# jgrss/cultionet

Hardware: AMD Instinct MI355X
Metric: train_chips_per_sec (higher is better)
Workload: dtype f32

## Files before the change

### cultionet_amd/csrc/cn_thin.hip

```cpp
#include "cn_common.h"

namespace {

struct Taps {
  int off[9];
  bool ok[9];
};

__device__ __forceinline__ Taps cn_thin_taps(int oy, int ox, int H, int W, int dil, int sgn) {
  Taps tp;
#pragma unroll
  for (int t = 0; t < 9; ++t) {
    const int iy = oy + sgn * (t / 3 - 1) * dil, ix = ox + sgn * (t % 3 - 1) * dil;
    tp.ok[t] = iy >= 0 && iy < H && ix >= 0 && ix < W;
    tp.off[t] = tp.ok[t] ? iy * W + ix : 0;
  }
  return tp;
}

#define CN_THIN_W(g) ((g) == 0 ? w0 : ((g) == 1 ? w1 : w2))
#define CN_THIN_B(g) ((g) == 0 ? b0 : ((g) == 1 ? b1 : b2))
#define CN_THIN_DW(g) ((g) == 0 ? dw0 : ((g) == 1 ? dw1 : dw2))

template <int NG, int CP, bool GROUPED>
// ... 262 lines not shown
#pragma unroll
    for (int u = 0; u < U; ++u) {
      if (c0 + u < Cq) {
        const int cw = wid * Cq + c0 + u;
        const float* wrow = wpk ? wpk + (long)(cw < Cin ? cw : 0) * RS : wl + cw * RS;
        const bool wok = !wpk || cw < Cin;
        const int wa = wok ? __float_as_int(wrow[lane]) : 0;
        const int wb = wok ? __float_as_int(wrow[64 + (lane < RS - 64 ? lane : 0)]) : 0;
#pragma unroll
        for (int o = 0; o < NO; ++o)
#pragma unroll
          for (int t = 0; t < 9; ++t) {
            const int i = o * 9 + t;
            acc[o] = fmaf(xv[u][t], __int_as_float(__builtin_amdgcn_readlane(i < 64 ? wa : wb, i & 63)), acc[o]);
          }
      }
    }
  }
#pragma unroll
  for (int o = 0; o < NO; ++o) red[(wid * NO + o) * 64 + lane] = acc[o];
  __syncthreads();
  for (int idx = threadIdx.x; idx < NO * 64; idx += 256) {
    const int o = idx >> 6, l = idx & 63;
    const int g = o / CP, c = o - g * CP;
    const float* bg = g == 0 ? b0 : (g == 1 ? b1 : b2);
    float v = bg != nullptr ? bg[c] : 0.f;
#pragma unroll
    for (int w = 0; w < 4; ++w) v += red[(w * NO + o) * 64 + l];
    const int p = bx * 64 + l;
    if (p < HW) y[(long)by * ybs + (long)o * HW + p] = v;
  }
}

template <int NG, int CP>
__global__ __launch_bounds__(256) void cn_thin_bwd_data_ks_kernel(const float* __restrict__ dy, long dybs,
                                                                 const float* __restrict__ w0,
                                                                 const float* __restrict__ w1,
                                                                 const float* __restrict__ w2,
                                                                 float* __restrict__ dx, long dxbs, int Cin, int H,
                                                                 int W, int dil, int accumulate, int Cq, int B,
                                                                 const float* __restrict__ wpk) {
  constexpr int NO = NG * CP, RS = (NO * 9 + 3) / 4 * 4;
  extern __shared__ __attribute__((aligned(16))) float sm[];
  float* wl = sm;
  const int lane = threadIdx.x & 63, wid = threadIdx.x >> 6;
  const int HW = H * W;
  int bx, by, bz;
  const int gx = (HW + 63) / 64;
  if (!cn_xcd_block(gx, B, gx * B, bx, by, bz)) return;
  const int pix = bx * 64 + lane;
  const bool live = pix < HW;
  const int pc = live ? pix : 0;
  const int oy = pc / W, ox = pc - oy * W;
  const Taps tp = cn_thin_taps(oy, ox, H, W, dil, -1);
  if (!wpk) cn_thin_stage_weights<NG, CP>(wl, Cq, Cin, w0, w1, w2);
  const float* dyb = dy + (long)by * dybs;
  f32x2 dv[RS / 2];
#pragma unroll
  for (int i = 0; i < RS; ++i) {
    const int o = i / 9, t = i - o * 9;
    const float v = (i < NO * 9 && tp.ok[t]) ? dyb[(long)o * HW + tp.off[t]] : 0.f;
    dv[i >> 1][i & 1] = v;
  }
  __syncthreads();
  float* dxb = dx + (long)by * dxbs + pix;
  for (int cil = 0; cil < Cq; ++cil) {
    const int ci = wid * Cq + cil;
    if (ci >= Cin) break;
    f32x2 s2[2] = {{0.f, 0.f}, {0.f, 0.f}};
    if (wpk) {
      const float* wr = wpk + (long)__builtin_amdgcn_readfirstlane(ci) * RS;
#pragma unroll
      for (int j = 0; j < RS / 2; ++j) {
        const f32x2 w2 = {wr[2 * j], wr[2 * j + 1]};
        s2[j & 1] = __builtin_elementwise_fma(dv[j], w2, s2[j & 1]);
      }
    } else {
    const float* wrow = wl + (wid * Cq + cil) * RS;
    const int wa = __float_as_int(wrow[lane]);
    const int wb = __float_as_int(wrow[64 + (lane < RS - 64 ? lane : 0)]);
#pragma unroll
    for (int j = 0; j < RS / 2; ++j) {
      const int i0 = 2 * j, i1 = 2 * j + 1;
      const f32x2 w2 = {__int_as_float(__builtin_amdgcn_readlane(i0 < 64 ? wa : wb, i0 & 63)),
                        __int_as_float(__builtin_amdgcn_readlane(i1 < 64 ? wa : wb, i1 & 63))};
      s2[j & 1] = __builtin_elementwise_fma(dv[j], w2, s2[j & 1]);
    }
    }
    const float r = (s2[0][0] + s2[0][1]) + (s2[1][0] + s2[1][1]);
    if (live) {
      float* d = dxb + (long)ci * HW;
      *d = accumulate ? *d + r : r;
    }
  }
}

int cn_thin_cfg(int nsets, int cout_per_set, int grouped) {
  if (nsets == 3 && cout_per_set == 3 && !grouped) return 0;
  if (nsets == 3 && cout_per_set == 1 && grouped) return 1;
  if (nsets == 1 && cout_per_set == 3 && !grouped) return 2;
  if (nsets == 1 && cout_per_set == 1 && !grouped) return 3;
  return -1;
}

}

#define CN_THIN_DISPATCH(cfg, CALL)        \
  switch (cfg) {                           \
    case 0: { CALL(3, 3, false); } break;  \
    case 1: { CALL(3, 1, true); } break;   \
    case 2: { CALL(1, 3, false); } break;  \
    default: { CALL(1, 1, false); } break; \
  }

extern "C" int cn_thin_conv3x3_fwd_f32(const float* x, long xbs, const float* const* ws, const float* const* biases,
                                       float* y, long ybs, int B, int Cin, int H, int W, int nsets, int cout_per_set,
                                       int grouped, int dil, float* wpack, void* stream) {
  const int cfg = cn_thin_cfg(nsets, cout_per_set, grouped);
  if (cfg < 0 || dil < 1 || Cin < 1) return CN_ERR_ARG;
  if (B <= 0 || H <= 0 || W <= 0) return CN_OK;
  const float* w[3] = {ws[0], nsets > 1 ? ws[1] : nullptr, nsets > 2 ? ws[2] : nullptr};
  const float* b[3] = {nullptr, nullptr, nullptr};
  if (biases)
    for (int i = 0; i < nsets; ++i) b[i] = biases[i];
  if (cfg == 0 && Cin >= 16) {
    const int Cq = (Cin + 3) / 4;
    const size_t lds = sizeof(float) * (size_t)((wpack ? 0 : 4 * Cq * 84) + 4 * 9 * 64);
    if (lds <= 64 * 1024) {
      if (wpack)
        CN_LAUNCH((cn_thin_pack_kernel<3, 3>), dim3(cn_cdiv((long)Cin * 84, 256)), dim3(256), 0,
                           (hipStream_t)stream, w[0], w[1], w[2], wpack, Cin);
      CN_LAUNCH((cn_thin_fwd_ks_kernel<3, 3>), dim3(cn_xcd_grid((long)cn_cdiv((long)H * W, 64) * B)), dim3(256), lds,
                         (hipStream_t)stream, x, xbs, w[0], w[1], w[2], b[0], b[1], b[2], y, ybs, Cin, H, W, dil, Cq, B,
                         (const float*)wpack);
      return cn_check_launch();
    }
  }
  const dim3 grid(cn_cdiv((long)H * W, 256), B);
#define CN_CALL(NG_, CP_, GR_)                                                                                      \
  CN_LAUNCH((cn_thin_fwd_kernel<NG_, CP_, GR_>), grid, dim3(256), 0, (hipStream_t)stream, x, xbs, w[0], w[1], \
                     w[2], b[0], b[1], b[2], y, ybs, Cin, H, W, dil)
  CN_THIN_DISPATCH(cfg, CN_CALL)
#undef CN_CALL
  return cn_check_launch();
}

extern "C" int cn_thin_conv3x3_bwd_data_f32(const float* dy, long dybs, const float* const* ws, float* dx, long dxbs,
                                            int B, int Cin, int H, int W, int nsets, int cout_per_set, int grouped,
                                            int dil, int accumulate, float* wpack, void* stream) {
  const int cfg = cn_thin_cfg(nsets, cout_per_set, grouped);
  if (cfg < 0 || dil < 1 || Cin < 1) return CN_ERR_ARG;
  if (B <= 0 || H <= 0 || W <= 0) return CN_OK;
  const float* w[3] = {ws[0], nsets > 1 ? ws[1] : nullptr, nsets > 2 ? ws[2] : nullptr};
  if (cfg == 0 && Cin >= 16) {
    const int Cq = (Cin + 3) / 4;
    const size_t lds = sizeof(float) * (size_t)(wpack ? 0 : 4 * Cq * 84);
    if (lds <= 64 * 1024) {
      if (wpack)
        CN_LAUNCH((cn_thin_pack_kernel<3, 3>), dim3(cn_cdiv((long)Cin * 84, 256)), dim3(256), 0,
                           (hipStream_t)stream, w[0], w[1], w[2], wpack, Cin);
      CN_LAUNCH((cn_thin_bwd_data_ks_kernel<3, 3>), dim3(cn_xcd_grid((long)cn_cdiv((long)H * W, 64) * B)), dim3(256), lds,
                         (hipStream_t)stream, dy, dybs, w[0], w[1], w[2], dx, dxbs, Cin, H, W, dil, accumulate, Cq, B,
                         (const float*)wpack);
      return cn_check_launch();
    }
  }
  const dim3 grid(cn_cdiv((long)H * W, 256), B);
#define CN_CALL(NG_, CP_, GR_)                                                                                   \
  CN_LAUNCH((cn_thin_bwd_data_kernel<NG_, CP_, GR_>), grid, dim3(256), 0, (hipStream_t)stream, dy, dybs, \
                     w[0], w[1], w[2], dx, dxbs, Cin, H, W, dil, accumulate)
  CN_THIN_DISPATCH(cfg, CN_CALL)
#undef CN_CALL
  return cn_check_launch();
}

extern "C" int cn_thin_conv3x3_bwd_weight_f32(const float* x, long xbs, const float* dy, long dybs, float* const* dws,
                                              int B, int Cin, int H, int W, int nsets, int cout_per_set, int grouped,
                                              int dil, void* stream) {
  const int cfg = cn_thin_cfg(nsets, cout_per_set, grouped);
  if (cfg < 0 || dil < 1 || Cin < 1) return CN_ERR_ARG;
  if (B <= 0 || H <= 0 || W <= 0) return CN_OK;
  float* dw[3] = {dws[0], nsets > 1 ? dws[1] : nullptr, nsets > 2 ? dws[2] : nullptr};
  const int cin_total = grouped ? nsets * Cin : Cin;
  const int col_tiles = (W + 127) / 128;
  const int R = B * H;
  int chunks = 1024 / (cin_total * col_tiles);
  if (chunks < 1) chunks = 1;
  int per = (R + chunks - 1) / chunks;
  if (per < 32) per = 32;
  per = (per + 1) & ~1;
  chunks = (R + per - 1) / per;
  const dim3 grid((unsigned)(chunks * col_tiles), cin_total);
#define CN_CALL(NG_, CP_, GR_)                                                                                      \
  CN_LAUNCH((cn_thin_bwd_weight_kernel<NG_, CP_, GR_>), grid, dim3(256), 0, (hipStream_t)stream, x, xbs, dy, \
                     dybs, dw[0], dw[1], dw[2], B, Cin, H, W, dil, per, col_tiles)
  CN_THIN_DISPATCH(cfg, CN_CALL)
#undef CN_CALL
  return cn_check_launch();
// ... 2 lines not shown
```

### cultionet_amd/csrc/cn_wgrad.hip

```cpp
#include <cstdlib>
#include "cn_common.h"
#include "cn_conv_geom.h"
#include "cn_profile.h"
#include "cn_slicesum.h"

#define WG_MAX_TAPS 9
#define WG_BC 32
#define WG_NS 4
#define WG_NB 13
#define WG_DS 32
#define WG_DB 64
#define WG_U 4

struct CnWgradGeom {
  int N;
  int A, Hs, Ws; long sbs; long scs;
  int Bc, Hb, Wb; long bbs; long bcs;
  double flops;
  int s;
  int T;
  int offy[WG_MAX_TAPS], offx[WG_MAX_TAPS];
  int min_oy, min_ox;
  long sa;
  int PR, Wsp, pitch_s;
  int rows_b, pitch_b, plane_b;
  int a_tiles;
  int chunks_per_img, total_chunks, chunks_per_split;
  int b_lds_off;
  int buf_stride;
  int nbuf;
  int colsplit;
  int G, spg;
  const float* gS[4];
  const float* gB[4];
  float* gdW[4];
  long slice_stride;
  int grid_x, grid_y, grid_z;
  int mq_lo, mq_hi;
};

typedef __attribute__((address_space(3))) void* cn_lds_ptr;
typedef const __attribute__((address_space(1))) void* cn_gbl_ptr;

__device__ float cn_zero_line[64];

__device__ __forceinline__ void cn_glds4(const float* src, float* lds_wave_base) {
  __builtin_amdgcn_global_load_lds((cn_gbl_ptr)src, (cn_lds_ptr)lds_wave_base, 4, 0, 0);
}

template <int T>
__global__ __launch_bounds__(256) void cn_wgrad_kernel(const float* __restrict__ S, const float* __restrict__ Bg,
                                                      float* __restrict__ dW, const CnWgradGeom g) {
  extern __shared__ __attribute__((aligned(16))) float smem[];

  const int tid = threadIdx.x, lane = tid & 63, wid = tid >> 6;
  const int half = lane >> 5, l31 = lane & 31;
  const int at = wid % g.a_tiles, kp = wid / g.a_tiles, kparts = 4 / g.a_tiles;
  int bx, by, bz;
  if (!cn_xcd_block(g.grid_x, g.grid_y, g.grid_x * g.grid_y * g.grid_z, bx, by, bz)) return;
  const int a0 = by * g.a_tiles * 32;
  const int b0 = bx * WG_BC;
  const int npix = g.PR * g.Wsp;
  const float* zero = cn_zero_line + lane;

  int so[WG_NS];
#pragma unroll
  for (int i = 0; i < WG_NS; ++i) {
    const int e = lane + i * 64;
    if (e < npix) {
      const int r = e / g.Wsp, c = e - r * g.Wsp;
      so[i] = (r << 16) | ((c < g.Ws) ? c : 0xFFFF);
    } else {
// ... 128 lines not shown
  static_assert(T == 1, "3 x 3 kernels run on cn_wgrad_vec3_kernel");
  constexpr int KR = 1;
#include "cn_wgrad_vec_body.h"
}

template <int S_>
__global__ __launch_bounds__(768) void cn_wgrad_vec3_kernel(const float* __restrict__ S0, const float* __restrict__ Bg0,
                                                           float* __restrict__ dW0, const CnWgradGeom g) {
  constexpr int KR = 3;
#include "cn_wgrad_vec_body.h"
}

struct CnWgradReduceArgs {
  const float* part; long slice_stride; int nslices; long n;
  float* dW[4];
};
__global__ __launch_bounds__(256) void cn_wgrad_reduce_kernel(const CnWgradReduceArgs a) {
  const long i = blockIdx.x * 256L + threadIdx.x;
  if (i >= a.n) return;
  const float* part = a.part + (long)blockIdx.z * a.nslices * a.slice_stride;
  float* dW = a.dW[blockIdx.z];
  float s0 = 0.f, s1 = 0.f;
  int k = blockIdx.y;
  for (; k + (int)gridDim.y < a.nslices; k += 2 * gridDim.y) {
    s0 += part[(long)k * a.slice_stride + i];
    s1 += part[(long)(k + gridDim.y) * a.slice_stride + i];
  }
  if (k < a.nslices) s0 += part[(long)k * a.slice_stride + i];
  if (gridDim.y == 1) dW[i] += s0 + s1;
  else atomicAdd(dW + i, s0 + s1);
}

template <int T>
static int cn_wgrad_launch_vec(const float* S, const float* Bg, float* dW, CnWgradGeom g, float* ws, long ws_floats,
                               hipStream_t stream) {
  if (g.scs % 4 || g.bcs % 4 || g.sbs % 4 || g.bbs % 4 || (g.Ws & 1)) return CN_ERR_ARG;
  g.Wsp = g.Ws;
  g.PR = 128 / g.Ws;
  if (g.PR < 1) g.PR = 1;
  if (g.PR > g.Hs) g.PR = g.Hs;
  while (g.PR > 1 && (g.PR * g.Ws) % 4 != 0) --g.PR;
  if ((g.PR * g.Ws) % 4 != 0 && g.Ws % 2 == 0 && 2 * g.Ws <= 256) g.PR = 2;
  if ((g.PR * g.Ws) % 4 != 0 || g.PR * g.Ws > 256) return CN_ERR_ARG;
  int max_oy = g.min_oy, max_ox = g.min_ox;
  for (int t = 0; t < g.T; ++t) {
    if (g.offy[t] > max_oy) max_oy = g.offy[t];
    if (g.offx[t] > max_ox) max_ox = g.offx[t];
  }
  g.rows_b = (g.PR - 1) * g.s + (max_oy - g.min_oy) + 1;
  g.pitch_b = g.Wb;
  g.plane_b = ((g.rows_b - 1) * g.Wb + (g.Ws - 1) * g.s + (max_ox - g.min_ox) + 4 + 3) / 4 * 4;
  if (WG_BC * g.plane_b > WG_DB * 256) return CN_ERR_ARG;
  g.pitch_s = g.PR * g.Ws;
  g.a_tiles = g.A > 32 ? 2 : 1;
  size_t lds;
  for (;;) {
    g.b_lds_off = (g.a_tiles * 32 * g.pitch_s + 255) / 256 * 256;
    g.buf_stride = g.b_lds_off + (WG_BC * g.plane_b + 255) / 256 * 256;
    lds = (size_t)g.buf_stride * sizeof(float);
    if ((lds <= 160 * 1024 && g.a_tiles * 32 * g.pitch_s <= WG_DS * 256) || g.a_tiles == 1) break;
    g.a_tiles >>= 1;
  }
  if (lds > 160 * 1024 || g.a_tiles * 32 * g.pitch_s > WG_DS * 256) return CN_ERR_ARG;
  g.nbuf = (2 * lds <= 160 * 1024) ? 2 : 1;
  lds *= g.nbuf;
  {
    const size_t red = (size_t)(4 / g.a_tiles - 1) * g.a_tiles * T * 16 * 64 * sizeof(float);
    if (red > lds) lds = red;
  }
  g.chunks_per_img = (g.Hs + g.PR - 1) / g.PR;
  g.total_chunks = g.N * g.chunks_per_img;
  const int gx = (g.Bc + WG_BC - 1) / WG_BC, gy = (g.A + g.a_tiles * 32 - 1) / (g.a_tiles * 32);
  if (g.G < 1) {
    g.G = 1;
    g.gS[0] = S; g.gB[0] = Bg; g.gdW[0] = dW;
  }
  for (int i = 0; i < g.G; ++i)
    if ((reinterpret_cast<uintptr_t>(g.gS[i]) & 15) || (reinterpret_cast<uintptr_t>(g.gB[i]) & 15)) return CN_ERR_ARG;
  const int slots = (lds * 2 <= 160 * 1024) ? 512 : 256;
  int splits = slots / (gx * gy * g.G);
  if (splits > g.total_chunks) splits = g.total_chunks;
  if (splits < 1) splits = 1;
  g.chunks_per_split = (g.total_chunks + splits - 1) / splits;
  splits = (g.total_chunks + g.chunks_per_split - 1) / g.chunks_per_split;
  if (g.s != 1 && g.s != 2) return CN_ERR_ARG;
  using Kern = void (*)(const float*, const float*, float*, CnWgradGeom);
  static const Kern kern[2] = {T == 9 ? cn_wgrad_vec3_kernel<1> : cn_wgrad_vec_kernel<1, 1>,
                               T == 9 ? cn_wgrad_vec3_kernel<2> : cn_wgrad_vec_kernel<1, 2>};
  static bool attr_set = false;
  if (!attr_set) {
    for (const Kern k : kern)
      (void)hipFuncSetAttribute((const void*)k, hipFuncAttributeMaxDynamicSharedMemorySize, 160 * 1024);
    attr_set = true;
  }
  {
    const int nq_row = g.Ws / 2;
    int lo = (-g.min_ox + 2 * g.s - 1) / (2 * g.s);
    if (lo < 0) lo = 0;
    int hi_num = g.Wb - max_ox - g.s;
    int hi = hi_num <= 0 ? 0 : (hi_num + 2 * g.s - 1) / (2 * g.s);
    if (lo > nq_row) lo = nq_row;
    if (hi > nq_row) hi = nq_row;
    if (hi < lo) hi = lo;
    g.mq_lo = lo;
    g.mq_hi = hi;
  }
  if (T == 9) cn_prof_name("cn_wgrad_vec3_kernel<%d>", g.s);
  else cn_prof_name("cn_wgrad_vec_kernel<1, %d>", g.s);
  g.spg = splits;
  g.grid_x = gx; g.grid_y = gy; g.grid_z = splits * g.G;
  const dim3 grid(cn_xcd_grid((long)gx * gy * splits * g.G));
  const int kparts = 4 / g.a_tiles;
  const long dw_floats = (long)g.A * g.sa;
  const long nslices = splits;
  float* out = g.gdW[0];
  g.slice_stride = 0;
  if (nslices >= 16 && ws != nullptr && nslices * g.G * dw_floats <= ws_floats) {
    g.slice_stride = dw_floats;
    out = ws;
  }
  cn_prof_desc("wgrad_vec<%d> G%d N%d A%d %dx%d Bc%d %dx%d s%d grid%dx%dx%d nbuf%d sl%d", T, g.G, g.N, g.A, g.Hs, g.Ws,
               g.Bc, g.Hb, g.Wb, g.s, gx, gy, splits, g.nbuf, g.slice_stride != 0 ? 1 : 0);
  cn_prof_bytes(4.0 * g.G * ((double)g.N * g.A * g.Hs * g.Ws + (double)g.N * g.Bc * g.Hb * g.Wb + (double)dw_floats));
  cn_prof_before(stream);
  CN_LAUNCH(kern[g.s - 1], grid, dim3(T == 9 ? 768 : 256), lds, stream, g.gS[0], g.gB[0], out, g);
  cn_prof_after(stream, T == 9 ? 2 : 3, g.flops * g.G);
  if (g.slice_stride != 0) {
    CnSliceSum js[4] = {};
    for (int i = 0; i < g.G; ++i) {
      js[i].part = ws + (long)i * nslices * g.slice_stride; js[i].dw = g.gdW[i]; js[i].slice_stride = g.slice_stride;
      js[i].n = dw_floats; js[i].nslices = (int)nslices; js[i].kind = 0;
    }
    if (cn_ss_push(js, g.G)) return cn_check_launch();
    CnWgradReduceArgs ra = {ws, g.slice_stride, (int)nslices, dw_floats, {g.gdW[0], g.gdW[1], g.gdW[2], g.gdW[3]}};
    CN_LAUNCH(cn_wgrad_reduce_kernel,
                       dim3((unsigned)((dw_floats + 255) / 256), nslices > 128 ? 16 : 1, g.G), dim3(256), 0, stream,
                       ra);
  }
  return cn_check_launch();
}

template <int T>
static int cn_wgrad_launch_t(const float* S, const float* Bg, float* dW, CnWgradGeom g, hipStream_t stream) {
  g.Wsp = (g.Ws + 1) & ~1;
  if (g.Wsp > 64 * WG_NS) return CN_ERR_LDS;
  g.PR = 128 / g.Wsp;
  if (g.PR < 1) g.PR = 1;
  if (g.PR > g.Hs) g.PR = g.Hs;
  int max_oy = g.min_oy, max_ox = g.min_ox;
  for (int t = 0; t < g.T; ++t) {
    if (g.offy[t] > max_oy) max_oy = g.offy[t];
    if (g.offx[t] > max_ox) max_ox = g.offx[t];
  }
  for (;;) {
    g.rows_b = (g.PR - 1) * g.s + (max_oy - g.min_oy) + 1;
    g.pitch_b = (g.Wsp - 1) * g.s + (max_ox - g.min_ox) + 1;
    g.plane_b = g.rows_b * g.pitch_b;
    if (g.plane_b <= 64 * WG_NB || g.PR == 1) break;
    --g.PR;
  }
  if (g.plane_b > 64 * WG_NB) return CN_ERR_LDS;
  g.pitch_s = (g.PR * g.Wsp) | 1;
  g.a_tiles = g.A > 64 ? 4 : (g.A > 32 ? 2 : 1);
  if (g.a_tiles == 4) g.a_tiles = 2;
  size_t lds;
  for (;;) {
    g.b_lds_off = (g.a_tiles * 32 * g.pitch_s + 3) / 4 * 4;
    g.buf_stride = (g.b_lds_off + WG_BC * g.plane_b + 3) / 4 * 4;
    lds = (size_t)g.buf_stride * sizeof(float);
    if (lds <= 160 * 1024 || g.a_tiles == 1) break;
    g.a_tiles >>= 1;
  }
// ... 89 lines not shown
  const bool ws_ok = ws != nullptr && (reinterpret_cast<uintptr_t>(ws) & 15) == 0;
  int rc = g.T == 1 ? cn_wgrad_launch_vec<1>(Ss[0], Bgs[0], dWs[0], g, ws_ok ? ws : nullptr, ws_floats, stream)
                    : cn_wgrad_launch_vec<9>(Ss[0], Bgs[0], dWs[0], g, ws_ok ? ws : nullptr, ws_floats, stream);
  if (rc != CN_ERR_ARG) return rc;
  if (ws_ok) {
    const int Wsp = (Ws + 1) & ~1;
    const long scs = ((long)Hs * Wsp + 3) / 4 * 4, bcs = ((long)Hb * Wb + 3) / 4 * 4;
    const long need_s = (long)N * A * scs, need_b = (long)N * Bc * bcs;
    CnWgradGeom gp = g;
    CnPadArgs pa = {};
    float* w = ws;
    long need = 0;
    bool any_s = false, any_b = false;
    for (int i = 0; i < G; ++i) {
      const bool s_ok = (g.scs % 4 == 0) && (sbs % 4 == 0) && !(Ws & 1) && !(reinterpret_cast<uintptr_t>(Ss[i]) & 15);
      const bool b_ok = (g.bcs % 4 == 0) && (bbs % 4 == 0) && !(reinterpret_cast<uintptr_t>(Bgs[i]) & 15);
      any_s |= !s_ok;
      any_b |= !b_ok;
    }
    for (int i = 0; i < G && any_s; ++i) {
      pa.set[pa.nsets++] = {Ss[i], sbs, (long)Hs * Ws, w, A, Hs, Ws, Wsp, (int)scs};
      gp.gS[i] = w; w += need_s; need += need_s;
    }
    for (int i = 0; i < G && any_b; ++i) {
      int same = -1;
      for (int j = 0; j < i; ++j)
        if (Bgs[j] == Bgs[i]) same = j;
      if (same >= 0) { gp.gB[i] = gp.gB[same]; continue; }
      pa.set[pa.nsets++] = {Bgs[i], bbs, (long)Hb * Wb, w, Bc, Hb, Wb, Wb, (int)bcs};
      gp.gB[i] = w; w += need_b; need += need_b;
    }
    if (any_s) { gp.Ws = Wsp; gp.scs = scs; gp.sbs = (long)A * scs; }
    if (any_b) { gp.bcs = bcs; gp.bbs = (long)Bc * bcs; }
    if (need <= ws_floats) {
      const int r = cn_pad_planes(pa, N, stream);
      if (r != CN_OK) return r;
      float* wrest = ws + (need + 3) / 4 * 4;
      const long nrest = ws_floats - (need + 3) / 4 * 4;
      rc = g.T == 1 ? cn_wgrad_launch_vec<1>(gp.gS[0], gp.gB[0], dWs[0], gp, wrest, nrest, stream)
                    : cn_wgrad_launch_vec<9>(gp.gS[0], gp.gB[0], dWs[0], gp, wrest, nrest, stream);
      if (rc != CN_ERR_ARG) return rc;
    }
  }
  for (int i = 0; i < G; ++i) {
    CnWgradGeom g1 = g;
    g1.G = 0;
    rc = g.T == 1 ? cn_wgrad_launch_t<1>(Ss[i], Bgs[i], dWs[i], g1, stream)
                  : cn_wgrad_launch_t<9>(Ss[i], Bgs[i], dWs[i], g1, stream);
    if (rc != CN_OK) return rc;
  }
  return CN_OK;
}

static int cn_wgrad_generic(const float* S, long sbs, int A, int Hs, int Ws, const float* Bg, long bbs, int Bc,
                            int Hb, int Wb, int s, int KH, int KW, int dil, int pad, float* dW, int N, float* ws,
                            long ws_floats, hipStream_t stream) {
  return cn_wgrad_generic_g(1, &S, sbs, A, Hs, Ws, &Bg, bbs, Bc, Hb, Wb, s, KH, KW, dil, pad, &dW, N, ws, ws_floats,
                            stream);
}

extern "C" int cn_conv2d_bwd_weight_grouped_f32(int G, const float* const* xs, long xbs, const float* const* dys,
                                                long dybs, float* const* dws, int B, int Cin, int Hin, int Win,
                                                int Cout, int KH, int KW, int stride, int pad, int dil, float* ws,
                                                long ws_floats, void* stream) {
  if (stride < 1) return CN_ERR_ARG;
  const int Hout = cn_conv_out(Hin, KH, stride, pad, dil);
  const int Wout = cn_conv_out(Win, KW, stride, pad, dil);
  return cn_wgrad_generic_g(G, dys, dybs, Cout, Hout, Wout, xs, xbs, Cin, Hin, Win, stride, KH, KW, dil, pad, dws, B,
                            ws, ws_floats, (hipStream_t)stream);
}

extern "C" int cn_conv2d_bwd_weight_f32(const float* x, long xbs, const float* dy, long dybs, float* dw, int B,
                                        int Cin, int Hin, int Win, int Cout, int KH, int KW, int stride, int pad,
                                        int dil, float* ws, long ws_floats, void* stream) {
// ... 18 lines not shown
```

### cultionet_amd/scratch.py

```python
from __future__ import annotations

import os
import struct
import typing as T

import torch

from . import _lib, runtime
from .params import _bump_ws_epoch
from .runtime import _main_stream, _py_op, _side_state, _state, _stream


_DEFER_SUMS = os.environ.get("CN_DEFER_SUMS", "1") != "0"
_SS_CAP = 512
_SS_BLOCK = 64 << 20
_SS_FLUSH_FLOATS = int(float(os.environ.get("CN_SUM_FLUSH_MB", "128")) * (1 << 20) / 4)


class _SliceSums:

    def __init__(self, dev: torch.device):
        self.dev = dev
        self.host = torch.zeros(_SS_CAP * 64, dtype=torch.uint8).pin_memory()
        self.table = torch.zeros(_SS_CAP * 64, dtype=torch.uint8, device=dev)
# ... 107 lines not shown
            del st.uploaded[k]
        st.uploaded[(first, n)] = now
        _py_op(st.upload_ev.record, sobj)
    st.pending = 0
    st.flushed = n
    st.cur, st.off = 0, 0



def _zeroed_scratch(n: int, dev: torch.device) -> torch.Tensor:
    ws = torch.empty(n, dtype=torch.float32, device=dev)
    _lib.call("cn_fill_f32", ws.data_ptr(), n, 0.0, _stream())
    return ws


def _grown(pool: T.Dict, key, need: int, dev: torch.device, zeroed: bool) -> torch.Tensor:
    ws = pool.get(key)
    if ws is None or ws.numel() < need:
        if ws is not None:
            torch.cuda.synchronize(dev)
        ws = pool[key] = _zeroed_scratch(need, dev) if zeroed else torch.empty(need, dtype=torch.float32, device=dev)
        _bump_ws_epoch()
    return ws


_WS_FLOATS = 16 << 20


def _pad_ws(*tensors: torch.Tensor) -> T.Tuple[T.Optional[int], int]:
    need = _WS_FLOATS
    for t in tensors:
        H, W = t.shape[-2], t.shape[-1]
        if (H * W) % 4 or (W & 1):
            need += t.shape[0] * t.shape[1] * (H * (W + 1) + 3)
    dev = tensors[0].device
    ss = _ss_state()
    if ss is not None:
        return ss.take(need)
    pool = _state.ws_pool
    if pool is None:
        pool = _state.ws_pool = {}
    ws = _grown(pool, dev, need, dev, zeroed=False)
    return ws.data_ptr(), ws.numel()


_pt_ws: T.Dict[T.Tuple, torch.Tensor] = {}


def _pretime_ws(need: int, dev: torch.device) -> torch.Tensor:
    return _grown(_pt_ws, (dev, _stream()), need, dev, zeroed=True)


_WS16_MAX_FLOATS = 96 << 20


def _ws16(need: int, dev: torch.device, pool_name: str = "wgrad") -> T.Tuple[int, int]:
    need = int(min(max(need, 1 << 20), _WS16_MAX_FLOATS))
    if pool_name == "wgrad":
        ss = _ss_state()
        if ss is not None:
            return ss.take(need)
    pool = _state.ws16_pool
    if pool is None:
        pool = _state.ws16_pool = {}
    key = (dev, pool_name) if pool_name in ("wgrad", "side") else (dev, pool_name, _state.stream_override)
    ws = _grown(pool, key, need, dev, zeroed=True)
    return ws.data_ptr(), ws.numel()
# ... 13 lines not shown
```

Before: 404.3.

## Rewrite thin conv backward-data as persistent MFMA kernel with prefetched tiles

Replaces the scalar-FMA backward-data kernel for the 3x3-set thin convolution with a persistent kernel built on 32x32x2 f32 MFMA instructions. Each wave keeps a 32-channel weight slice in registers and walks pixel tiles in a strided stream, using buffer loads with out-of-bounds offsets for zero padding. It prefetches the next tile's dy operands while the current MFMAs run. The weight-pack path is dropped and accumulate becomes a template parameter. The trade-offs are higher register pressure, padding waste when Cin is not a multiple of 32, and a fixed grid sized around 2048 waves.

```diff
diff --git a/cultionet_amd/csrc/cn_thin.hip b/cultionet_amd/csrc/cn_thin.hip
--- a/cultionet_amd/csrc/cn_thin.hip
+++ b/cultionet_amd/csrc/cn_thin.hip
@@ -318,66 +318,119 @@
   }
 }
 
-template <int NG, int CP>
-__global__ __launch_bounds__(256) void cn_thin_bwd_data_ks_kernel(const float* __restrict__ dy, long dybs,
-                                                                 const float* __restrict__ w0,
-                                                                 const float* __restrict__ w1,
-                                                                 const float* __restrict__ w2,
-                                                                 float* __restrict__ dx, long dxbs, int Cin, int H,
-                                                                 int W, int dil, int accumulate, int Cq, int B,
-                                                                 const float* __restrict__ wpk) {
-  constexpr int NO = NG * CP, RS = (NO * 9 + 3) / 4 * 4;
-  extern __shared__ __attribute__((aligned(16))) float sm[];
-  float* wl = sm;
-  const int lane = threadIdx.x & 63, wid = threadIdx.x >> 6;
+template <int NG, int CP, bool ACC>
+__global__ __launch_bounds__(256) void cn_thin_bwd_data_mfma_kernel(const float* __restrict__ dy, long dybs,
+                                                                   const float* __restrict__ w0,
+                                                                   const float* __restrict__ w1,
+                                                                   const float* __restrict__ w2,
+                                                                   float* __restrict__ dx, long dxbs, int Cin, int H,
+                                                                   int W, int dil, int nct, int nstreams,
+                                                                   int tiles_per_img, int ntiles, int nblocks) {
+  constexpr int NO = NG * CP, K = NO * 9, KS = (K + 1) / 2;
+  constexpr unsigned OOB = 0x80000000u;
+  __shared__ float wl[4][NO * 288];
+  int lb, by_, bz_;
+  if (!cn_xcd_block(nblocks, 1, nblocks, lb, by_, bz_)) return;
+  const int wid = __builtin_amdgcn_readfirstlane((int)(threadIdx.x >> 6));
+  const int gw = lb * 4 + wid;
+  if (gw >= nct * nstreams) return;
+  const int stream = gw / nct, ct = gw - stream * nct;
+  if (stream >= ntiles) return;
+  const int lane = threadIdx.x & 63, h = lane >> 5, j = lane & 31;
   const int HW = H * W;
-  int bx, by, bz;
-  const int gx = (HW + 63) / 64;
-  if (!cn_xcd_block(gx, B, gx * B, bx, by, bz)) return;
-  const int pix = bx * 64 + lane;
-  const bool live = pix < HW;
-  const int pc = live ? pix : 0;
-  const int oy = pc / W, ox = pc - oy * W;
-  const Taps tp = cn_thin_taps(oy, ox, H, W, dil, -1);
-  if (!wpk) cn_thin_stage_weights<NG, CP>(wl, Cq, Cin, w0, w1, w2);
-  const float* dyb = dy + (long)by * dybs;
-  f32x2 dv[RS / 2];
-#pragma unroll
-  for (int i = 0; i < RS; ++i) {
-    const int o = i / 9, t = i - o * 9;
-    const float v = (i < NO * 9 && tp.ok[t]) ? dyb[(long)o * HW + tp.off[t]] : 0.f;
-    dv[i >> 1][i & 1] = v;
-  }
-  __syncthreads();
-  float* dxb = dx + (long)by * dxbs + pix;
-  for (int cil = 0; cil < Cq; ++cil) {
-    const int ci = wid * Cq + cil;
-    if (ci >= Cin) break;
-    f32x2 s2[2] = {{0.f, 0.f}, {0.f, 0.f}};
-    if (wpk) {
-      const float* wr = wpk + (long)__builtin_amdgcn_readfirstlane(ci) * RS;
-#pragma unroll
-      for (int j = 0; j < RS / 2; ++j) {
-        const f32x2 w2 = {wr[2 * j], wr[2 * j + 1]};
-        s2[j & 1] = __builtin_elementwise_fma(dv[j], w2, s2[j & 1]);
+
+  float a[KS];
+  {
+    float* wv = wl[wid];
+#pragma unroll
+    for (int o = 0; o < NO; ++o) {
+      const float* wg = CN_THIN_W(o / CP) + (long)(o % CP) * Cin * 9;
+#pragma unroll
+      for (int i0 = 0; i0 < 288; i0 += 64) {
+        const int i = i0 + lane;
+        const int cl = i / 9, t = i - cl * 9;
+        const int ch = ct * 32 + cl < Cin ? ct * 32 + cl : Cin - 1;
+        if (i < 288) wv[o * 288 + i] = wg[(long)ch * 9 + t];
       }
-    } else {
-    const float* wrow = wl + (wid * Cq + cil) * RS;
-    const int wa = __float_as_int(wrow[lane]);
-    const int wb = __float_as_int(wrow[64 + (lane < RS - 64 ? lane : 0)]);
-#pragma unroll
-    for (int j = 0; j < RS / 2; ++j) {
-      const int i0 = 2 * j, i1 = 2 * j + 1;
-      const f32x2 w2 = {__int_as_float(__builtin_amdgcn_readlane(i0 < 64 ? wa : wb, i0 & 63)),
-                        __int_as_float(__builtin_amdgcn_readlane(i1 < 64 ? wa : wb, i1 & 63))};
-      s2[j & 1] = __builtin_elementwise_fma(dv[j], w2, s2[j & 1]);
-    }
-    }
-    const float r = (s2[0][0] + s2[0][1]) + (s2[1][0] + s2[1][1]);
-    if (live) {
-      float* d = dxb + (long)ci * HW;
-      *d = accumulate ? *d + r : r;
-    }
+    }
+    __builtin_amdgcn_wave_barrier();
+#pragma unroll
+    for (int s = 0; s < KS; ++s) {
+      const int k0 = 2 * s, k1 = (2 * s + 1 < K) ? 2 * s + 1 : k0;
+      const int i0 = (k0 / 9) * 288 + k0 % 9, i1 = (k1 / 9) * 288 + k1 % 9;
+      const float v = wv[(h ? i1 : i0) + 9 * j];
+      a[s] = __int_as_float(__float_as_int(v) & ((2 * s + 1 < K) ? -1 : h - 1));
+    }
+  }
+  long chofs[16];
+#pragma unroll
+  for (int r = 0; r < 16; ++r) {
+    const int ch = ct * 32 + (r & 3) + 8 * (r >> 2) + 4 * h;
+    chofs[r] = (long)(ch < Cin ? ch : Cin - 1) * HW;
+  }
+
+  struct TileB {
+    __amdgpu_buffer_rsrc_t rs;
+    unsigned voff[11];
+  };
+  auto tile_b = [&](int tile) {
+    TileB tb;
+    const int b = tile / tiles_per_img, pt = tile - b * tiles_per_img;
+    const int pix = pt * 32 + j < HW ? pt * 32 + j : HW - 1;
+    const int oy = pix / W, ox = pix - oy * W;
+    const Taps tp = cn_thin_taps(oy, ox, H, W, dil, -1);
+#pragma unroll
+    for (int q = 0; q < 9; ++q) {
+      const int t0 = (2 * q) % 9, t1 = (2 * q + 1) % 9;
+      const bool ok = h ? tp.ok[t1] : tp.ok[t0];
+      tb.voff[q] = ok ? (unsigned)(h ? tp.off[t1] : tp.off[t0]) * 4u : OOB;
+    }
+    tb.voff[9] = (h == 0 && tp.ok[8]) ? (unsigned)tp.off[8] * 4u : OOB;
+    tb.voff[10] = tb.voff[4] + (h ? (unsigned)HW * 4u : 0u);
+    tb.rs = __builtin_amdgcn_make_buffer_rsrc(const_cast<float*>(dy + (long)b * dybs), 0, 0x7fffffff, 0x00020000);
+    return tb;
+  };
+  auto load_b = [&](const TileB& tb, int s) {
+    const int k0 = 2 * s, k1 = (2 * s + 1 < K) ? 2 * s + 1 : k0;
+    const int q = 2 * s + 1 >= K ? 9 : (k1 / 9 != k0 / 9 ? 10 : s % 9);
+    return __builtin_bit_cast(float, __builtin_amdgcn_raw_buffer_load_b32(tb.rs, tb.voff[q], (k0 / 9) * HW * 4, 0));
+  };
+
+  float bv[KS];
+  int tile = stream;
+  TileB cur = tile_b(tile);
+#pragma unroll
+  for (int s = 0; s < KS; ++s) bv[s] = load_b(cur, s);
+  for (;;) {
+    const int nt = tile + nstreams;
+    const bool more = nt < ntiles;
+    const TileB nxt = tile_b(more ? nt : tile);
+    f32x16 acc;
+#pragma unroll
+    for (int r = 0; r < 16; ++r) acc[r] = 0.f;
+#pragma unroll
+    for (int s = 0; s < KS; ++s) {
+      acc = __builtin_amdgcn_mfma_f32_32x32x2f32(a[s], bv[s], acc, 0, 0, 0);
+      bv[s] = load_b(nxt, s);
+      __builtin_amdgcn_sched_barrier(0);
+    }
+    {
+      const int b = tile / tiles_per_img, pt = tile - b * tiles_per_img;
+      const int pix = pt * 32 + j < HW ? pt * 32 + j : HW - 1;
+      float* dxb = dx + (long)b * dxbs + pix;
+      if (ACC) {
+        float old[16];
+#pragma unroll
+        for (int r = 0; r < 16; ++r) old[r] = dxb[chofs[r]];
+#pragma unroll
+        for (int r = 0; r < 16; ++r) acc[r] += old[r];
+      }
+#pragma unroll
+      for (int r = 0; r < 16; ++r) dxb[chofs[r]] = acc[r];
+    }
+    if (!more) break;
+    tile = nt;
+    cur = nxt;
   }
 }
 
@@ -438,18 +491,25 @@
   if (cfg < 0 || dil < 1 || Cin < 1) return CN_ERR_ARG;
   if (B <= 0 || H <= 0 || W <= 0) return CN_OK;
   const float* w[3] = {ws[0], nsets > 1 ? ws[1] : nullptr, nsets > 2 ? ws[2] : nullptr};
-  if (cfg == 0 && Cin >= 16) {
-    const int Cq = (Cin + 3) / 4;
-    const size_t lds = sizeof(float) * (size_t)(wpack ? 0 : 4 * Cq * 84);
-    if (lds <= 64 * 1024) {
-      if (wpack)
-        CN_LAUNCH((cn_thin_pack_kernel<3, 3>), dim3(cn_cdiv((long)Cin * 84, 256)), dim3(256), 0,
-                           (hipStream_t)stream, w[0], w[1], w[2], wpack, Cin);
-      CN_LAUNCH((cn_thin_bwd_data_ks_kernel<3, 3>), dim3(cn_xcd_grid((long)cn_cdiv((long)H * W, 64) * B)), dim3(256), lds,
-                         (hipStream_t)stream, dy, dybs, w[0], w[1], w[2], dx, dxbs, Cin, H, W, dil, accumulate, Cq, B,
-                         (const float*)wpack);
-      return cn_check_launch();
-    }
+  (void)wpack;
+  const long tiles = (long)cn_cdiv((long)H * W, 32) * B;
+  if (cfg == 0 && Cin >= 16 && (long)H * W <= (1l << 25) && tiles < (1l << 30)) {
+    const int nct = cn_cdiv(Cin, 32);
+    int nstreams = 2048 / nct;
+    if (nstreams < 1) nstreams = 1;
+    nstreams = cn_cdiv(tiles, cn_cdiv(tiles, nstreams));
+    const int nblocks = cn_cdiv((long)nct * nstreams, 4);
+#define CN_CALL(ACC_)                                                                                          \
+  CN_LAUNCH((cn_thin_bwd_data_mfma_kernel<3, 3, ACC_>), dim3(cn_xcd_grid(nblocks)), dim3(256), 0,              \
+            (hipStream_t)stream, dy, dybs, w[0], w[1], w[2], dx, dxbs, Cin, H, W, dil, nct, nstreams,          \
+            cn_cdiv((long)H * W, 32), (int)tiles, nblocks)
+    if (accumulate) {
+      CN_CALL(true);
+    } else {
+      CN_CALL(false);
+    }
+#undef CN_CALL
+    return cn_check_launch();
   }
   const dim3 grid(cn_cdiv((long)H * W, 256), B);
 #define CN_CALL(NG_, CP_, GR_)                                                                                   \
```

Measured after the change: 404.8 (median of 5 runs). About the same (+0.1%).

## Add flattened-plane layout path for weight-gradient kernel on padded inputs

Applied to the files above, without the earlier changes.

Splits wgrad planning into a reusable header and adds a 'flat' mode. In this mode each input plane is padded with a horizontal halo and treated as one 1-D row, and taps become linear offsets. It is used only when the padded path would otherwise run and the flat plan matches the row plan's grid, splits and tiling. The aim is to cut wasted lanes and odd-width handling for planes whose width does not fit the vectorised row layout. The cost is extra padding work, a larger workspace and extra halo compute.

```diff
diff --git a/cultionet_amd/csrc/cn_wgrad.hip b/cultionet_amd/csrc/cn_wgrad.hip
--- a/cultionet_amd/csrc/cn_wgrad.hip
+++ b/cultionet_amd/csrc/cn_wgrad.hip
@@ -3,41 +3,7 @@
 #include "cn_conv_geom.h"
 #include "cn_profile.h"
 #include "cn_slicesum.h"
-
-#define WG_MAX_TAPS 9
-#define WG_BC 32
-#define WG_NS 4
-#define WG_NB 13
-#define WG_DS 32
-#define WG_DB 64
-#define WG_U 4
-
-struct CnWgradGeom {
-  int N;
-  int A, Hs, Ws; long sbs; long scs;
-  int Bc, Hb, Wb; long bbs; long bcs;
-  double flops;
-  int s;
-  int T;
-  int offy[WG_MAX_TAPS], offx[WG_MAX_TAPS];
-  int min_oy, min_ox;
-  long sa;
-  int PR, Wsp, pitch_s;
-  int rows_b, pitch_b, plane_b;
-  int a_tiles;
-  int chunks_per_img, total_chunks, chunks_per_split;
-  int b_lds_off;
-  int buf_stride;
-  int nbuf;
-  int colsplit;
-  int G, spg;
-  const float* gS[4];
-  const float* gB[4];
-  float* gdW[4];
-  long slice_stride;
-  int grid_x, grid_y, grid_z;
-  int mq_lo, mq_hi;
-};
+#include "cn_wgrad_geom.h"
 
 typedef __attribute__((address_space(3))) void* cn_lds_ptr;
 typedef const __attribute__((address_space(1))) void* cn_gbl_ptr;
@@ -232,58 +198,10 @@
 }
 
 template <int T>
-static int cn_wgrad_launch_vec(const float* S, const float* Bg, float* dW, CnWgradGeom g, float* ws, long ws_floats,
-                               hipStream_t stream) {
-  if (g.scs % 4 || g.bcs % 4 || g.sbs % 4 || g.bbs % 4 || (g.Ws & 1)) return CN_ERR_ARG;
-  g.Wsp = g.Ws;
-  g.PR = 128 / g.Ws;
-  if (g.PR < 1) g.PR = 1;
-  if (g.PR > g.Hs) g.PR = g.Hs;
-  while (g.PR > 1 && (g.PR * g.Ws) % 4 != 0) --g.PR;
-  if ((g.PR * g.Ws) % 4 != 0 && g.Ws % 2 == 0 && 2 * g.Ws <= 256) g.PR = 2;
-  if ((g.PR * g.Ws) % 4 != 0 || g.PR * g.Ws > 256) return CN_ERR_ARG;
-  int max_oy = g.min_oy, max_ox = g.min_ox;
-  for (int t = 0; t < g.T; ++t) {
-    if (g.offy[t] > max_oy) max_oy = g.offy[t];
-    if (g.offx[t] > max_ox) max_ox = g.offx[t];
-  }
-  g.rows_b = (g.PR - 1) * g.s + (max_oy - g.min_oy) + 1;
-  g.pitch_b = g.Wb;
-  g.plane_b = ((g.rows_b - 1) * g.Wb + (g.Ws - 1) * g.s + (max_ox - g.min_ox) + 4 + 3) / 4 * 4;
-  if (WG_BC * g.plane_b > WG_DB * 256) return CN_ERR_ARG;
-  g.pitch_s = g.PR * g.Ws;
-  g.a_tiles = g.A > 32 ? 2 : 1;
-  size_t lds;
-  for (;;) {
-    g.b_lds_off = (g.a_tiles * 32 * g.pitch_s + 255) / 256 * 256;
-    g.buf_stride = g.b_lds_off + (WG_BC * g.plane_b + 255) / 256 * 256;
-    lds = (size_t)g.buf_stride * sizeof(float);
-    if ((lds <= 160 * 1024 && g.a_tiles * 32 * g.pitch_s <= WG_DS * 256) || g.a_tiles == 1) break;
-    g.a_tiles >>= 1;
-  }
-  if (lds > 160 * 1024 || g.a_tiles * 32 * g.pitch_s > WG_DS * 256) return CN_ERR_ARG;
-  g.nbuf = (2 * lds <= 160 * 1024) ? 2 : 1;
-  lds *= g.nbuf;
-  {
-    const size_t red = (size_t)(4 / g.a_tiles - 1) * g.a_tiles * T * 16 * 64 * sizeof(float);
-    if (red > lds) lds = red;
-  }
-  g.chunks_per_img = (g.Hs + g.PR - 1) / g.PR;
-  g.total_chunks = g.N * g.chunks_per_img;
-  const int gx = (g.Bc + WG_BC - 1) / WG_BC, gy = (g.A + g.a_tiles * 32 - 1) / (g.a_tiles * 32);
-  if (g.G < 1) {
-    g.G = 1;
-    g.gS[0] = S; g.gB[0] = Bg; g.gdW[0] = dW;
-  }
+static int cn_wgrad_launch_planned(CnWgradGeom g, const CnWgradPlan& p, int dHs, int dWs, int dHb, int dWb, int flat,
+                                   float* ws, hipStream_t stream) {
   for (int i = 0; i < g.G; ++i)
     if ((reinterpret_cast<uintptr_t>(g.gS[i]) & 15) || (reinterpret_cast<uintptr_t>(g.gB[i]) & 15)) return CN_ERR_ARG;
-  const int slots = (lds * 2 <= 160 * 1024) ? 512 : 256;
-  int splits = slots / (gx * gy * g.G);
-  if (splits > g.total_chunks) splits = g.total_chunks;
-  if (splits < 1) splits = 1;
-  g.chunks_per_split = (g.total_chunks + splits - 1) / splits;
-  splits = (g.total_chunks + g.chunks_per_split - 1) / g.chunks_per_split;
-  if (g.s != 1 && g.s != 2) return CN_ERR_ARG;
   using Kern = void (*)(const float*, const float*, float*, CnWgradGeom);
   static const Kern kern[2] = {T == 9 ? cn_wgrad_vec3_kernel<1> : cn_wgrad_vec_kernel<1, 1>,
                                T == 9 ? cn_wgrad_vec3_kernel<2> : cn_wgrad_vec_kernel<1, 2>};
@@ -293,37 +211,18 @@
       (void)hipFuncSetAttribute((const void*)k, hipFuncAttributeMaxDynamicSharedMemorySize, 160 * 1024);
     attr_set = true;
   }
-  {
-    const int nq_row = g.Ws / 2;
-    int lo = (-g.min_ox + 2 * g.s - 1) / (2 * g.s);
-    if (lo < 0) lo = 0;
-    int hi_num = g.Wb - max_ox - g.s;
-    int hi = hi_num <= 0 ? 0 : (hi_num + 2 * g.s - 1) / (2 * g.s);
-    if (lo > nq_row) lo = nq_row;
-    if (hi > nq_row) hi = nq_row;
-    if (hi < lo) hi = lo;
-    g.mq_lo = lo;
-    g.mq_hi = hi;
-  }
   if (T == 9) cn_prof_name("cn_wgrad_vec3_kernel<%d>", g.s);
   else cn_prof_name("cn_wgrad_vec_kernel<1, %d>", g.s);
-  g.spg = splits;
-  g.grid_x = gx; g.grid_y = gy; g.grid_z = splits * g.G;
-  const dim3 grid(cn_xcd_grid((long)gx * gy * splits * g.G));
-  const int kparts = 4 / g.a_tiles;
+  const int splits = p.splits;
+  const dim3 grid(cn_xcd_grid((long)p.gx * p.gy * splits * g.G));
   const long dw_floats = (long)g.A * g.sa;
   const long nslices = splits;
-  float* out = g.gdW[0];
-  g.slice_stride = 0;
-  if (nslices >= 16 && ws != nullptr && nslices * g.G * dw_floats <= ws_floats) {
-    g.slice_stride = dw_floats;
-    out = ws;
-  }
-  cn_prof_desc("wgrad_vec<%d> G%d N%d A%d %dx%d Bc%d %dx%d s%d grid%dx%dx%d nbuf%d sl%d", T, g.G, g.N, g.A, g.Hs, g.Ws,
-               g.Bc, g.Hb, g.Wb, g.s, gx, gy, splits, g.nbuf, g.slice_stride != 0 ? 1 : 0);
-  cn_prof_bytes(4.0 * g.G * ((double)g.N * g.A * g.Hs * g.Ws + (double)g.N * g.Bc * g.Hb * g.Wb + (double)dw_floats));
+  float* out = p.slices ? ws : g.gdW[0];
+  cn_prof_desc("wgrad_vec<%d> G%d N%d A%d %dx%d Bc%d %dx%d s%d grid%dx%dx%d nbuf%d sl%d fl%d", T, g.G, g.N, g.A, dHs, dWs,
+               g.Bc, dHb, dWb, g.s, p.gx, p.gy, splits, g.nbuf, p.slices, flat);
+  cn_prof_bytes(4.0 * g.G * ((double)g.N * g.A * dHs * dWs + (double)g.N * g.Bc * dHb * dWb + (double)dw_floats));
   cn_prof_before(stream);
-  CN_LAUNCH(kern[g.s - 1], grid, dim3(T == 9 ? 768 : 256), lds, stream, g.gS[0], g.gB[0], out, g);
+  CN_LAUNCH(kern[g.s - 1], grid, dim3(T == 9 ? 768 : 256), p.lds, stream, g.gS[0], g.gB[0], out, g);
   cn_prof_after(stream, T == 9 ? 2 : 3, g.flops * g.G);
   if (g.slice_stride != 0) {
     CnSliceSum js[4] = {};
@@ -338,6 +237,18 @@
                        ra);
   }
   return cn_check_launch();
+}
+
+template <int T>
+static int cn_wgrad_launch_vec(const float* S, const float* Bg, float* dW, CnWgradGeom g, float* ws, long ws_floats,
+                               hipStream_t stream) {
+  if (g.G < 1) {
+    g.G = 1;
+    g.gS[0] = S; g.gB[0] = Bg; g.gdW[0] = dW;
+  }
+  CnWgradPlan p;
+  if (!cn_wgrad_vec_rows(g) || !cn_wgrad_vec_plan(g, T, ws != nullptr, ws_floats, 0, p)) return CN_ERR_ARG;
+  return cn_wgrad_launch_planned<T>(g, p, g.Hs, g.Ws, g.Hb, g.Wb, 0, ws, stream);
 }
 
 template <int T>
@@ -493,14 +404,50 @@
     }
     if (any_s) { gp.Ws = Wsp; gp.scs = scs; gp.sbs = (long)A * scs; }
     if (any_b) { gp.bcs = bcs; gp.bbs = (long)Bc * bcs; }
-    if (need <= ws_floats) {
-      const int r = cn_pad_planes(pa, N, stream);
-      if (r != CN_OK) return r;
-      float* wrest = ws + (need + 3) / 4 * 4;
-      const long nrest = ws_floats - (need + 3) / 4 * 4;
-      rc = g.T == 1 ? cn_wgrad_launch_vec<1>(gp.gS[0], gp.gB[0], dWs[0], gp, wrest, nrest, stream)
-                    : cn_wgrad_launch_vec<9>(gp.gS[0], gp.gB[0], dWs[0], gp, wrest, nrest, stream);
-      if (rc != CN_ERR_ARG) return rc;
+    CnWgradPlan rp;
+    float* wrest = ws + (need + 3) / 4 * 4;
+    const long nrest = ws_floats - (need + 3) / 4 * 4;
+    if (need <= ws_floats && cn_wgrad_vec_rows(gp) && cn_wgrad_vec_plan(gp, g.T, true, nrest, 0, rp)) {
+      const long cs = cn_wgrad_flat_stride(Hs, Ws, cn_wgrad_flat_halo(g));
+      const int P = Ws + cn_wgrad_flat_halo(g);
+      const long fneed_s = (long)N * A * cs, fneed_b = (long)N * Bc * cs;
+      CnWgradGeom gf;
+      CnWgradPlan fp;
+      CnPadArgs pf = {};
+      long fneed = 0;
+      for (int i = 0; i < G; ++i) fneed += fneed_s;
+      for (int i = 0; i < G; ++i) {
+        bool dup = false;
+        for (int j = 0; j < i; ++j) dup |= Bgs[j] == Bgs[i];
+        if (!dup) fneed += fneed_b;
+      }
+      if (any_s && any_b && fneed <= ws_floats &&
+          cn_wgrad_flat_choose(g, g.T, gp, rp, true, ws_floats - fneed, gf, fp)) {
+        float* wf = ws;
+        for (int i = 0; i < G; ++i) {
+          pf.set[pf.nsets++] = {Ss[i], sbs, (long)Hs * Ws, wf, A, Hs, Ws, P, (int)cs};
+          gf.gS[i] = wf; wf += fneed_s;
+        }
+        for (int i = 0; i < G; ++i) {
+          int same = -1;
+          for (int j = 0; j < i; ++j)
+            if (Bgs[j] == Bgs[i]) same = j;
+          if (same >= 0) { gf.gB[i] = gf.gB[same]; continue; }
+          pf.set[pf.nsets++] = {Bgs[i], bbs, (long)Hb * Wb, wf, Bc, Hb, Wb, P, (int)cs};
+          gf.gB[i] = wf; wf += fneed_b;
+        }
+        const int r = cn_pad_planes(pf, N, stream);
+        if (r != CN_OK) return r;
+        rc = g.T == 1 ? cn_wgrad_launch_planned<1>(gf, fp, gp.Hs, gp.Ws, gp.Hb, gp.Wb, 1, ws + fneed, stream)
+                      : cn_wgrad_launch_planned<9>(gf, fp, gp.Hs, gp.Ws, gp.Hb, gp.Wb, 1, ws + fneed, stream);
+        if (rc != CN_ERR_ARG) return rc;
+      } else {
+        const int r = cn_pad_planes(pa, N, stream);
+        if (r != CN_OK) return r;
+        rc = g.T == 1 ? cn_wgrad_launch_planned<1>(gp, rp, gp.Hs, gp.Ws, gp.Hb, gp.Wb, 0, wrest, stream)
+                      : cn_wgrad_launch_planned<9>(gp, rp, gp.Hs, gp.Ws, gp.Hb, gp.Wb, 0, wrest, stream);
+        if (rc != CN_ERR_ARG) return rc;
+      }
     }
   }
   for (int i = 0; i < G; ++i) {
diff --git a/cultionet_amd/csrc/cn_wgrad_geom.h b/cultionet_amd/csrc/cn_wgrad_geom.h
--- /dev/null
+++ b/cultionet_amd/csrc/cn_wgrad_geom.h
@@ -0,0 +1,168 @@
+#pragma once
+#include <cstddef>
+
+#define WG_MAX_TAPS 9
+#define WG_BC 32
+#define WG_NS 4
+#define WG_NB 13
+#define WG_DS 32
+#define WG_DB 64
+#define WG_U 4
+
+struct CnWgradGeom {
+  int N;
+  int A, Hs, Ws; long sbs; long scs;
+  int Bc, Hb, Wb; long bbs; long bcs;
+  double flops;
+  int s;
+  int T;
+  int offy[WG_MAX_TAPS], offx[WG_MAX_TAPS];
+  int min_oy, min_ox;
+  long sa;
+  int PR, Wsp, pitch_s;
+  int rows_b, pitch_b, plane_b;
+  int a_tiles;
+  int chunks_per_img, total_chunks, chunks_per_split;
+  int b_lds_off;
+  int buf_stride;
+  int nbuf;
+  int colsplit;
+  int G, spg;
+  const float* gS[4];
+  const float* gB[4];
+  float* gdW[4];
+  long slice_stride;
+  int grid_x, grid_y, grid_z;
+  int mq_lo, mq_hi;
+};
+
+struct CnWgradPlan {
+  int gx, gy, splits;
+  int slots;
+  size_t lds;
+  int slices;
+};
+
+static inline bool cn_wgrad_vec_rows(CnWgradGeom& g) {
+  if (g.scs % 4 || g.bcs % 4 || g.sbs % 4 || g.bbs % 4 || (g.Ws & 1)) return false;
+  if (g.s != 1 && g.s != 2) return false;
+  g.Wsp = g.Ws;
+  g.PR = 128 / g.Ws;
+  if (g.PR < 1) g.PR = 1;
+  if (g.PR > g.Hs) g.PR = g.Hs;
+  while (g.PR > 1 && (g.PR * g.Ws) % 4 != 0) --g.PR;
+  if ((g.PR * g.Ws) % 4 != 0 && g.Ws % 2 == 0 && 2 * g.Ws <= 256) g.PR = 2;
+  if ((g.PR * g.Ws) % 4 != 0 || g.PR * g.Ws > 256) return false;
+  int max_oy = g.min_oy, max_ox = g.min_ox;
+  for (int t = 0; t < g.T; ++t) {
+    if (g.offy[t] > max_oy) max_oy = g.offy[t];
+    if (g.offx[t] > max_ox) max_ox = g.offx[t];
+  }
+  g.rows_b = (g.PR - 1) * g.s + (max_oy - g.min_oy) + 1;
+  g.pitch_b = g.Wb;
+  g.plane_b = ((g.rows_b - 1) * g.Wb + (g.Ws - 1) * g.s + (max_ox - g.min_ox) + 4 + 3) / 4 * 4;
+  g.pitch_s = g.PR * g.Ws;
+  g.chunks_per_img = (g.Hs + g.PR - 1) / g.PR;
+  const int nq_row = g.Ws / 2;
+  int lo = (-g.min_ox + 2 * g.s - 1) / (2 * g.s);
+  if (lo < 0) lo = 0;
+  int hi_num = g.Wb - max_ox - g.s;
+  int hi = hi_num <= 0 ? 0 : (hi_num + 2 * g.s - 1) / (2 * g.s);
+  if (lo > nq_row) lo = nq_row;
+  if (hi > nq_row) hi = nq_row;
+  if (hi < lo) hi = lo;
+  g.mq_lo = lo;
+  g.mq_hi = hi;
+  return true;
+}
+
+static inline int cn_wgrad_flat_halo(const CnWgradGeom& g) {
+  int h = 0;
+  for (int t = 0; t < g.T; ++t) {
+    const int a = g.offx[t] < 0 ? -g.offx[t] : g.offx[t];
+    if (a > h) h = a;
+  }
+  return h;
+}
+static inline long cn_wgrad_flat_stride(int H, int W, int h) { return ((long)H * (W + h) + 3) / 4 * 4; }
+static inline int cn_wgrad_lds_pitch(int n) { return n % 8 == 0 ? n + 4 : n; }
+static inline int cn_wgrad_flat_len(int H, int W, int h, int chunks) {
+  const int hp = H * (W + h);
+  return cn_wgrad_lds_pitch(((hp + chunks - 1) / chunks + 3) / 4 * 4);
+}
+
+static inline bool cn_wgrad_vec_flat(CnWgradGeom& g, int L) {
+  if (g.s != 1 || g.Hs != g.Hb || g.Ws != g.Wb || g.T < 1) return false;
+  if (L < 4 || L % 4 != 0 || L > 256) return false;
+  const int H = g.Hs, W = g.Ws, h = cn_wgrad_flat_halo(g), P = W + h;
+  const long cs = cn_wgrad_flat_stride(H, W, h);
+  int mn = 0, mx = 0;
+  for (int t = 0; t < g.T; ++t) {
+    const int o = g.offy[t] * P + g.offx[t];
+    g.offy[t] = 0;
+    g.offx[t] = o;
+    if (t == 0 || o < mn) mn = o;
+    if (t == 0 || o > mx) mx = o;
+  }
+  g.min_oy = 0; g.min_ox = mn;
+  g.scs = cs; g.sbs = (long)g.A * cs;
+  g.bcs = cs; g.bbs = (long)g.Bc * cs;
+  g.Ws = g.Wb = g.Wsp = L;
+  g.PR = 1;
+  g.pitch_s = L;
+  g.rows_b = 1;
+  g.pitch_b = L;
+  g.plane_b = cn_wgrad_lds_pitch((L - 1 + (mx - mn) + 4 + 3) / 4 * 4);
+  g.chunks_per_img = (H * P + L - 1) / L;
+  g.mq_lo = 0;
+  g.mq_hi = L / 2;
+  return true;
+}
+
+static inline bool cn_wgrad_vec_plan(CnWgradGeom& g, int T, bool have_ws, long ws_floats, int slots, CnWgradPlan& p) {
+  if (g.pitch_s % 4 != 0 || g.pitch_s > 256) return false;
+  if (WG_BC * g.plane_b > WG_DB * 256) return false;
+  g.a_tiles = g.A > 32 ? 2 : 1;
+  size_t lds;
+  for (;;) {
+    g.b_lds_off = (g.a_tiles * 32 * g.pitch_s + 255) / 256 * 256;
+    g.buf_stride = g.b_lds_off + (WG_BC * g.plane_b + 255) / 256 * 256;
+    lds = (size_t)g.buf_stride * sizeof(float);
+    if ((lds <= 160 * 1024 && g.a_tiles * 32 * g.pitch_s <= WG_DS * 256) || g.a_tiles == 1) break;
+    g.a_tiles >>= 1;
+  }
+  if (lds > 160 * 1024 || g.a_tiles * 32 * g.pitch_s > WG_DS * 256) return false;
+  g.nbuf = (2 * lds <= 160 * 1024) ? 2 : 1;
+  lds *= g.nbuf;
+  {
+    const size_t red = (size_t)(4 / g.a_tiles - 1) * g.a_tiles * T * 16 * 64 * sizeof(float);
+    if (red > lds) lds = red;
+  }
+  g.total_chunks = g.N * g.chunks_per_img;
+  const int G = g.G < 1 ? 1 : g.G;
+  const int gx = (g.Bc + WG_BC - 1) / WG_BC, gy = (g.A + g.a_tiles * 32 - 1) / (g.a_tiles * 32);
+  if (slots == 0) slots = (lds * 2 <= 160 * 1024) ? 512 : 256;
+  int splits = slots / (gx * gy * G);
+  if (splits > g.total_chunks) splits = g.total_chunks;
+  if (splits < 1) splits = 1;
+  g.chunks_per_split = (g.total_chunks + splits - 1) / splits;
+  splits = (g.total_chunks + g.chunks_per_split - 1) / g.chunks_per_split;
+  g.spg = splits;
+  g.grid_x = gx; g.grid_y = gy; g.grid_z = splits * G;
+  const long dw_floats = (long)g.A * g.sa;
+  p.slices = (splits >= 16 && have_ws && (long)splits * G * dw_floats <= ws_floats) ? 1 : 0;
+  g.slice_stride = p.slices ? dw_floats : 0;
+  p.gx = gx; p.gy = gy; p.splits = splits; p.slots = slots; p.lds = lds;
+  return true;
+}
+
+static inline bool cn_wgrad_flat_choose(const CnWgradGeom& tru, int T, const CnWgradGeom& row, const CnWgradPlan& rp,
+                                        bool have_ws, long ws_floats, CnWgradGeom& fl, CnWgradPlan& fp) {
+  fl = tru;
+  if (fl.s != 1 || fl.Hs != fl.Hb || fl.Ws != fl.Wb) return false;
+  const int L = cn_wgrad_flat_len(fl.Hs, fl.Ws, cn_wgrad_flat_halo(fl), row.chunks_per_img);
+  if (!cn_wgrad_vec_flat(fl, L) || fl.chunks_per_img != row.chunks_per_img) return false;
+  if (!cn_wgrad_vec_plan(fl, T, have_ws, ws_floats, rp.slots, fp)) return false;
+  return fl.a_tiles == row.a_tiles && fl.nbuf == row.nbuf && fp.gx == rp.gx && fp.gy == rp.gy &&
+         fp.splits == rp.splits && fp.slices == rp.slices;
+}
diff --git a/cultionet_amd/scratch.py b/cultionet_amd/scratch.py
--- a/cultionet_amd/scratch.py
+++ b/cultionet_amd/scratch.py
@@ -163,7 +163,7 @@
     for t in tensors:
         H, W = t.shape[-2], t.shape[-1]
         if (H * W) % 4 or (W & 1):
-            need += t.shape[0] * t.shape[1] * (H * (W + 1) + 3)
+            need += t.shape[0] * t.shape[1] * (H * (W + 2) + 3)
     dev = tensors[0].device
     ss = _ss_state()
     if ss is not None:
```

Result: faster. 402.6 before, 407.6 after, median of 5 (+1.2%).
